# PFLeget/treegp

Measured on AMD Instinct MI355X. Metric: GP solve+predict throughput, 2-D AnisotropicRBF N=65536, higher is better.
Workload: dtype f64

## Files before the change

treegp_amd/csrc/api.hip:

```cpp
#include "tgp_internal.h"

#include <chrono>

namespace {
struct Arena {
    char *base;
    size_t off = 0;
    template <typename T> T *take(size_t count) {
        T *p = reinterpret_cast<T *>(base + off);
        off += (count * sizeof(T) + 255) / 256 * 256;
        return p;
    }
};

struct Staging {
    void *buf = nullptr;
    size_t bytes = 0;
};
Staging g_dummy;
}

struct tgp_ctx_ext {
    Staging io;
    Staging hio;
// ... 321 lines not shown
    double *d_out = (double *)ext_of(ctx)->io.buf;
    rc = launch_unpack_lower(ctx, d_A, Np, n, d_out);
    if (rc) return rc;
    TGP_HIP(hipMemcpyAsync(out, d_out, (size_t)n * n * sizeof(double), hipMemcpyDeviceToHost, ctx->stream));
    TGP_HIP(hipStreamSynchronize(ctx->stream));
    return 0;
}

int tgp_factor_device(tgp_ctx *ctx, const tgp_factor *f, const double **d_A, const double **d_W, int64_t *Np) {
    TGP_ARG(f && d_A && d_W && Np);
    *d_A = f->d_A;
    *d_W = f->d_W;
    *Np = f->Np;
    return 0;
}

static int factor_and_solve(tgp_ctx *ctx, int64_t n, int64_t Np, const double *d_y, double *d_alpha, double *logdet,
                            double *ydota, tgp_factor **keep, bool augmented) {
    hipStream_t st = ctx->stream;
    tgp_ctx_ext *e = ext_of(ctx);
    double *d_A = e->A_cache, *d_W = e->W_cache;
    double *d_b = (double *)ctx->scratch;
    int rc = 0;
    static const bool both_sweeps = getenv("TGP_CHI2_BOTH_SWEEPS") != nullptr;
    const bool forward_only = d_alpha == nullptr && !both_sweeps;
    double *own_slabs = nullptr;
    int own_S = 0;
    auto fail = [&](int code) {
        if (own_slabs) (void)hipFree(own_slabs);
        return code;
    };
    static const bool dbg = getenv("TGP_HOST_PHASES") != nullptr;
    const auto h0 = std::chrono::steady_clock::now();
    int info = launch_potrf(ctx, d_A, Np, d_W, true, n);
    if (info < 0) return fail(info);
    const auto h1 = std::chrono::steady_clock::now();
    TGP_HIP(hipEventRecord(ctx->ev[2], st));
    double sweeps = 0.0;
    if (info == 0 && augmented) {
        rc = launch_logdet_rowsq(ctx, d_A, Np, n, ctx->d_scal);
        if (rc) return fail(rc);
        if (d_alpha) {
            int Sa = 0;
            (void)potrs_big_step(Np, &Sa);
            rc = tgp_ensure_scratch2(ctx, (size_t)Np * sizeof(double));
            if (rc) return fail(rc);
            double *d_z = (double *)ctx->scratch2, *slabs = nullptr;
            bool build = false;
            rc = acquire_slabs(ctx, Np, Sa, nullptr, nullptr, &slabs, &build);
            if (rc) return fail(rc);
            rc = launch_vslab_build(ctx, d_A, d_W, Np, Sa, slabs);
            if (rc) return fail(rc);
            rc = launch_extract_row(ctx, d_A, Np, n, d_z);
            if (rc) return fail(rc);
            rc = launch_potrs_big_bwd(ctx, d_A, Np, Sa, slabs, d_b, d_z);
            if (rc) return fail(rc);
            sweeps = 1.0;
            TGP_HIP(hipMemcpyAsync(d_alpha, d_b, (size_t)n * sizeof(double), hipMemcpyDeviceToDevice, st));
        }
        TGP_HIP(hipMemcpyAsync(ctx->h_scal, ctx->d_scal, 2 * sizeof(double), hipMemcpyDeviceToHost, st));
    } else if (info == 0) {
        rc = launch_pad_copy(ctx, d_y, n, Np, d_b);
        if (rc) return fail(rc);
        int S2 = 0;
        if (keep && !own_slabs && potrs_big_step(Np, &S2) && ctx->vslab && ctx->vslab_bytes == vslab_bytes(Np, S2)) {
            own_slabs = (double *)ctx->vslab;
            own_S = S2;
            ctx->vslab = nullptr;
            ctx->vslab_bytes = 0;
        }
        if (own_slabs) {
            rc = launch_vslab_build(ctx, d_A, d_W, Np, own_S, own_slabs);
            if (rc) return fail(rc);
        }
        rc = launch_potrs(ctx, d_A, d_W, Np, d_b, forward_only, keep ? &own_slabs : nullptr, keep ? &own_S : nullptr);
        if (rc) return fail(rc);
        sweeps = forward_only ? 1.0 : 2.0;
        rc = launch_logdet_dot(ctx, d_A, Np, n, forward_only ? d_b : d_y, d_b, ctx->d_scal);
        if (rc) return fail(rc);
        if (d_alpha) TGP_HIP(hipMemcpyAsync(d_alpha, d_b, (size_t)n * sizeof(double), hipMemcpyDeviceToDevice, st));
        TGP_HIP(hipMemcpyAsync(ctx->h_scal, ctx->d_scal, 2 * sizeof(double), hipMemcpyDeviceToHost, st));
    }
    TGP_HIP(hipEventRecord(ctx->ev[3], st));
    const auto h2 = std::chrono::steady_clock::now();
    TGP_HIP(hipStreamSynchronize(st));
    if (dbg) {
        const auto h3 = std::chrono::steady_clock::now();
        auto d = [](std::chrono::steady_clock::time_point a, std::chrono::steady_clock::time_point b) { return std::chrono::duration<double, std::milli>(b - a).count(); };
        fprintf(stderr, "[factor_and_solve] launch_potrf returned after %.2f ms, solves queued after %.2f ms, final sync %.2f ms\n", d(h0, h1), d(h1, h2), d(h2, h3));
    }
    if (info == 0) info = *ctx->h_info;
    if (info < 0) return fail(tgp_potrf_info_rc(ctx, info));
    float ms = 0.f;
    TGP_HIP(hipEventElapsedTime(&ms, ctx->ev[0], ctx->ev[1]));
    ctx->timings[0] = ms;
    TGP_HIP(hipEventElapsedTime(&ms, ctx->ev[1], ctx->ev[2]));
    ctx->timings[1] = ms;
    TGP_HIP(hipEventElapsedTime(&ms, ctx->ev[2], ctx->ev[3]));
    ctx->timings[2] = ms;
    ctx->timings[8] = 8.0 * ((double)Np * (Np + 1) / 2.0) + 16.0 * (double)Np;
    ctx->timings[10] = sweeps;
    if (info > 0) {
        if (info > n) info = (int)n;
        return fail(info);
    }
    if (logdet) *logdet = ctx->h_scal[0];
    if (ydota) *ydota = ctx->h_scal[1];
    if (keep) {
        tgp_factor *f = new tgp_factor();
        f->n = n;
        f->Np = Np;
        f->d_A = d_A;
        f->d_W = d_W;
        f->d_slabs = own_slabs;
        f->slab_S = own_S;
        e->A_cache = e->W_cache = nullptr;
        e->cache_Np = 0;
        *keep = f;
    }
    return 0;
}

static int gp_solve_once(tgp_ctx *ctx, const tgp_kernel *k, const double *d_X, int64_t n, const double *d_y,
                         const double *d_yerr, double *d_alpha, double *logdet, double *ydota, tgp_factor **keep);
int tgp_d_gp_solve(tgp_ctx *ctx, const tgp_kernel *k, const double *d_X, int64_t n, const double *d_y,
                   const double *d_yerr, double *d_alpha, double *logdet, double *ydota, tgp_factor **keep) {
    SolveInFlight here;
    ctx->mid_allowed = here.alone ? 1 : 0;
    int rc = gp_solve_once(ctx, k, d_X, n, d_y, d_yerr, d_alpha, logdet, ydota, keep);
    ctx->mid_allowed = 0;
    if (rc == TGP_RC_HANDOFF && !ctx->mid_off) {
        ctx->mid_off = 1;
        rc = gp_solve_once(ctx, k, d_X, n, d_y, d_yerr, d_alpha, logdet, ydota, keep);
    }
    return rc;
}
// ... 298 lines not shown
```

treegp_amd/csrc/chol.hip:

```cpp
#include "tgp_internal.h"

#include "gemm_tile.h"
#include "potrf128.h"

#ifdef TGP_POTRF_STAMPS
__device__ unsigned long long tgp_gemm_stamps[1024 * 4];
__device__ int tgp_gemm_stamp_grid = 43;
__device__ unsigned long long tgp_queue_stamps[1024 * 4];
__device__ int tgp_queue_stamp_T = 40;
__device__ unsigned long long tgp_mid_stamps[25 * 8];
__device__ int tgp_mid_stamp_base = 5120;
#define TGP_MID_STAMP(i)                                                                                   \
    do {                                                                                                   \
        if (threadIdx.x == 0 && base == tgp_mid_stamp_base && blockIdx.x < 25) tgp_mid_stamps[blockIdx.x * 8 + (i)] = __builtin_amdgcn_s_memrealtime(); \
    } while (0)
#else
#define TGP_MID_STAMP(i) ((void)0)
#endif

namespace {
template <int MODE, int LDB>
__global__ __launch_bounds__(256, 2) void gemm_col_kernel(const double *A, const double *B, double *C) {
    const int64_t t = blockIdx.x;
    TGP_CHAIN_PRIO();
// ... 556 lines not shown
    static const int strip32_t = [] { const char *e = getenv("TGP_STRIP32_T"); return e ? atoi(e) : 64; }();
    if (strip > 0 && T <= strip32_t) {
        syrk_strip32_kernel<NSEG><<<(unsigned)((int64_t)4 * T * strip), 256, 0, st>>>(d_A, Np, ob, T, strip, P0, P1);
        return;
    }
    if (strip > 0 && T <= strip64_t) {
        syrk_strip64_kernel<NSEG><<<(unsigned)((int64_t)2 * T * strip), 256, 0, st>>>(d_A, Np, ob, T, strip, P0, P1);
        return;
    }
    const unsigned gs = strip == 0 ? (unsigned)tilemap_grid(T) : (unsigned)((int64_t)T * strip);
    syrk_dtv_kernel<NSEG><<<gs, 256, 0, st>>>(d_A, Np, ob, T, strip, P0, P1);
}

int queued_nres(int T) {
    static const int queue_res = [] { const char *e = getenv("TGP_QUEUE_RES"); return e ? atoi(e) : 0; }();
    if (queue_res > 0) return queue_res > TGP_QUEUE_MAXRES ? TGP_QUEUE_MAXRES : queue_res;
    static const int t1 = [] { const char *e = getenv("TGP_QUEUE_T1"); return e ? atoi(e) : 42; }();
    static const int t2 = [] { const char *e = getenv("TGP_QUEUE_T2"); return e ? atoi(e) : 26; }();
    return T >= t1 ? 1 : (T >= t2 ? 2 : 3);
}
void launch_syrk2_queued(tgp_ctx *ctx, hipStream_t st, double *d_A, int64_t Np, int ob, int T, const double *P0, const double *P1,
                         int nqueue) {
    const int nres = queued_nres(T);
    static const int half_env = [] { const char *e = getenv("TGP_QUEUE_HALF"); return e ? atoi(e) : -1; }();
    const unsigned slots = (unsigned)(tilemap_grid(T) / 8);
    unsigned nhalf = half_env >= 0 ? (unsigned)half_env : (unsigned)(512 - 64 * nres) / 8u;
    if (nhalf > slots) nhalf = slots;
    static const int steal = [] { const char *e = getenv("TGP_QUEUE_STEAL"); return e ? atoi(e) : 1; }();
    syrk_dtv_queue_kernel<2><<<512 + 8, 256, 0, st>>>(d_A, Np, ob, T, slots + nhalf, slots - nhalf, nres,
                                                     ctx->d_queue + TGP_QUEUE_WORDS * nqueue, P0, P1, steal);
}
}

int launch_potrf(tgp_ctx *ctx, double *d_A, int64_t Np, double *d_W, bool defer_info, int64_t n_data) {
    TGP_ARG(Np > 0 && Np % TGP_PW == 0);
    hipStream_t st = ctx->stream;
    TGP_HIP(hipMemsetAsync(ctx->d_info, 0, sizeof(int), st));
    const int nP = (int)(Np / TGP_PW);
    const bool prof = ctx->profiling != 0;
    if (prof) {
        while ((int)ctx->prof_events.size() < 2 * nP) {
            hipEvent_t e;
            TGP_HIP(hipEventCreate(&e));
            ctx->prof_events.push_back(e);
        }
    }
    static const int mode_env = [] { const char *e = getenv("TGP_CHOL_MODE"); return e ? atoi(e) : -1; }();
    const int mode = mode_env >= 0 ? mode_env : (!ctx->lookahead ? 1 : (Np >= 18432 ? 3 : (Np <= 1280 ? 1 : 2)));
    if (mode >= 2) {
        int rc = tgp_ensure_side_stream(ctx);
        if (rc) return rc;
    }
    double flops = 0.0;
    int nlaunch = 0;
    bool counting = true;
    auto timed = [&](auto &&fn, double fl) -> int {
        if (!counting) {
            fn();
            return 0;
        }
        if (prof) TGP_HIP(hipEventRecord(ctx->prof_events[2 * nlaunch], st));
        fn();
        if (prof) TGP_HIP(hipEventRecord(ctx->prof_events[2 * nlaunch + 1], st));
        flops += fl;
        ++nlaunch;
        return 0;
    };
    auto Wk = [&](int k) { return d_W + (int64_t)(2 * k) * TGP_TB * TGP_TB; };
// ... 109 lines not shown
                    syrk_small_kernel<2><<<dim3((unsigned)(T * 8), (unsigned)cols), 256, 0, st>>>(
                        d_A, Np, ob, T, seg_rows(k0 + i, ob), seg_rows(k0 + i + 1, ob));
                return;
            }
            SegPtrs<4> P{{seg_rows(k0, ob), seg_rows(k0 + 1, ob), seg_rows(k0 + 2, ob), seg_rows(k0 + 3, ob)},
                         {nullptr, nullptr, nullptr, nullptr}};
            const unsigned gs = strip == 0 ? (unsigned)tilemap_grid(T) : (unsigned)((int64_t)T * strip);
            syrk_segs_kernel<4><<<gs, 256, 0, st>>>(d_A, Np, ob, T, strip, P);
        };
        static const int tail_tiles = [] { const char *e = getenv("TGP_QUAD_TAIL_TILES"); return e ? atoi(e) : 96; }();
        factor_group(st, 0);
        for (int k = 0; k + 4 < nP; k += 4) {
            const int T4 = (int)((Np - (int64_t)TGP_PW * (k + 4)) / TGP_TB);
            if (T4 <= tail_tiles) {
                const double m = (double)T4 * TGP_TB;
                int rc = timed([&] { bulk(k, k + 4, T4, 0); }, 4.0 * TGP_PW * m * (m + 1.0));
                if (rc) return rc;
                counting = false;
                rc = run_pairs(k + 4);
                counting = true;
                if (rc) return rc;
                break;
            }
            {
                const double rows = (double)T4 * TGP_TB, w = (T4 < 8 ? T4 : 8) * (double)TGP_TB;
                const double elems = w * (rows - w) + w * (w + 1.0) / 2.0;
                int rc = timed([&] { bulk(k, k + 4, T4, 8); }, 2.0 * 4.0 * TGP_PW * elems);
                if (rc) return rc;
            }
            TGP_HIP(tgp_signal(ctx, st, 0, ctx->ev[4]));
            TGP_HIP(tgp_await(ctx, sd, 0, ctx->ev[4]));
            factor_group(sd, k + 4);
            TGP_HIP(tgp_signal(ctx, sd, 1, ctx->ev[5]));
            const int T5 = T4 - 8;
            if (T5 > 0) {
                const double m = (double)T5 * TGP_TB;
                int rc = timed([&] { bulk(k, k + 8, T5, 0); }, 4.0 * TGP_PW * m * (m + 1.0));
                if (rc) return rc;
            }
            TGP_HIP(tgp_await(ctx, st, 1, ctx->ev[5]));
        }
    } else if (mode == 2) {
        int rc = run_pairs(0);
        if (rc) return rc;
    } else {
        for (int k = 0; k < nP; k += 2) {
            const int64_t mk = Np - (int64_t)TGP_PW * k;
            factor_panel(st, panel(k), mk, Wk(k), ctx->d_info, k * TGP_PW, false, n_data, psync(k), 256);
            if (k + 1 >= nP) break;
            const int T1 = (int)((mk - TGP_PW) / TGP_TB);
            launch_syrk<1>(st, d_A, Np, k + 1, T1, 2, panel(k) + (int64_t)TGP_PW * TGP_PW, nullptr);
            factor_panel(st, panel(k + 1), mk - TGP_PW, Wk(k + 1), ctx->d_info, (k + 1) * TGP_PW, false, n_data, psync(k + 1), 256);
            const int T2 = T1 - 2;
            if (T2 > 0) {
                const double m = (double)T2 * TGP_TB;
                int rc = timed([&] { launch_syrk<2>(st, d_A, Np, k + 2, T2, 0, panel(k) + (int64_t)2 * TGP_PW * TGP_PW,
                                                     panel(k + 1) + (int64_t)TGP_PW * TGP_PW); },
                               2.0 * TGP_PW * m * (m + 1.0));
                if (rc) return rc;
            }
        }
    }
    TGP_HIP(hipGetLastError());
    TGP_HIP(hipMemcpyAsync(ctx->h_info, ctx->d_info, sizeof(int), hipMemcpyDeviceToHost, st));
    ctx->timings[6] = nlaunch;
    ctx->timings[7] = flops;
    ctx->timings[5] = 0.0;
    if (defer_info && !prof) return 0;
    TGP_HIP(hipStreamSynchronize(st));
    if (prof) {
        double tot = 0.0;
        for (int i = 0; i < nlaunch; ++i) {
            float ms = 0.f;
// ... 213 lines not shown
```

treegp_amd/csrc/tgp_internal.h:

```cpp
#pragma once
#include <hip/hip_runtime.h>
#include <cstdint>
#include <cstdio>
#include <cstdlib>
#include <cstring>
#include <string>
#include <atomic>
#include <vector>
#include "../../include/tgp.h"

#ifdef TGP_NO_CHAIN_PRIO
#define TGP_CHAIN_PRIO() ((void)0)
#else
#define TGP_CHAIN_PRIO() __builtin_amdgcn_s_setprio(3)
#endif

#define TGP_QUEUE_MAXRES 6
#define TGP_QUEUE_LEAVE (8 + 32 * TGP_QUEUE_MAXRES)
#define TGP_QUEUE_WORDS (TGP_QUEUE_LEAVE + 8)
#define TGP_NQUEUE 128
#define TGP_PSYNC_PANELS 1024
#define TGP_TB 128
#define TGP_PW 256
#define TGP_VAR_CHUNK_MAX 65280
// ... 117 lines not shown
    const int64_t S = (T + (1 << sh) - 1) >> sh;
    const int64_t ns = S * (S + 1) / 2;
    const int per = 1 << (2 * sh), q = per >= 8 ? per / 8 : 1;
    const int xcd = (int)(b & 7);
    const int64_t slot = b >> 3;
    const int64_t whole = (ns / 8) * per;
    int64_t st;
    int within;
    if (slot < whole) {
        st = (slot >> (2 * sh)) * 8 + xcd;
        within = (int)(slot & (per - 1));
    } else {
        const int64_t nn = slot - whole;
        st = (ns / 8) * 8 + nn / q;
        within = xcd * q + (int)(nn % q);
        if (st >= ns || within >= per) return;
    }
    int64_t Si, Sj;
    tri_index(st, Si, Sj);
    const int i = (int)((Si << sh) + (within >> sh));
    const int j = (int)((Sj << sh) + (within & ((1 << sh) - 1)));
    if (j > i || i >= T) return;
    ti = i; tj = j;
}

int tgp_ensure_side_stream(tgp_ctx *ctx);
int tgp_ensure_scratch(tgp_ctx *ctx, size_t bytes);
int tgp_ensure_scratch2(tgp_ctx *ctx, size_t bytes);
int tgp_ensure_pinned(tgp_ctx *ctx, size_t bytes, void **out);
int launch_kbuild_lower(tgp_ctx *ctx, const tgp_kernel *k, const double *d_X, int64_t n, int64_t Np,
                        const double *d_yerr, double *d_A);
int launch_kernel_dense(tgp_ctx *ctx, const tgp_kernel *k, const double *d_X, int64_t n,
                        const double *d_Y, int64_t m, int self, double *d_out);
int launch_potrf(tgp_ctx *ctx, double *d_A, int64_t Np, double *d_W, bool defer_info = false, int64_t n_data = -1);
int tgp_potrf_info_rc(tgp_ctx *ctx, int info);
#define TGP_RC_HANDOFF (-4)
extern std::atomic<int> tgp_solves_in_flight;
#define TGP_FLAG_HEAD 8
#define TGP_FLAG_HEAD_COUNT 9
bool tgp_handoff_by_flags(tgp_ctx *ctx);
unsigned tgp_next_seq(tgp_ctx *ctx, int id, hipError_t *err);
hipError_t tgp_signal_value(tgp_ctx *ctx, hipStream_t from, int id, unsigned v);
hipError_t tgp_signal(tgp_ctx *ctx, hipStream_t from, int id, hipEvent_t ev);
hipError_t tgp_await(tgp_ctx *ctx, hipStream_t to, int id, hipEvent_t ev);
bool potrs_big_step(int64_t Np, int *S);
int acquire_slabs(tgp_ctx *ctx, int64_t Np, int S, double **slab_cache, int *slab_S, double **out, bool *need_build);
int launch_potrs_big_bwd(tgp_ctx *ctx, const double *d_A, int64_t Np, int S, const double *slabs, double *d_b, double *d_z);
int launch_kbuild_lower_dist(tgp_ctx *ctx, const tgp_kernel *k, const double *d_X, int64_t n, int64_t Np,
                             const double *d_yerr, double *d_Aloc, const int64_t *d_loff, int G, int g);
int launch_factor_diag256(tgp_ctx *ctx, double *blk, double *W0, double *W1, int base, bool latency = false);
int launch_trsm_rows(tgp_ctx *ctx, double *rows, int ntiles, const double *Lkk, const double *W0, const double *W1, double *keepW = nullptr);
int launch_syrk_distn(tgp_ctx *ctx, double *d_Aloc, const int64_t *d_loff, int64_t Np, int kpanel, int G, int g, int nseg,
                      const double *const *d_P, const int *cmax, int col_lo, int col_hi, int queue_nres = 0, int head_cols = 0,
                      const double *const *d_PB = nullptr);
int launch_diag256_fwd(tgp_ctx *ctx, const double *Lkk, const double *W0, const double *W1, double *y);
int launch_diag256_bwd(tgp_ctx *ctx, const double *Lkk, const double *W0, const double *W1, double *y, const double *s);
int launch_fwd_update_rows(tgp_ctx *ctx, const double *Lrows, int64_t rows, const double *z, double *yrows);
int launch_gemv_t_rows(tgp_ctx *ctx, const double *Lrows, int64_t rows, const double *a, double *s, int64_t max_rows);
int launch_logdet_dist(tgp_ctx *ctx, const double *d_Aloc, const int64_t *d_loff, int64_t Np, int64_t n, int G, int g,
                       double *d_out);
int launch_potrs(tgp_ctx *ctx, const double *d_A, const double *d_W, int64_t Np, double *d_b, bool forward_only = false,
                 double **slab_cache = nullptr, int *slab_S = nullptr);
int launch_potrs_128(tgp_ctx *ctx, const double *d_A, const double *d_W, int64_t Np, double *d_b, bool forward_only);
size_t vslab_bytes(int64_t Np, int S);
int factor_slabs(tgp_ctx *ctx, tgp_factor *f, int want_S, int *S, const double **slabs);
int tgp_ensure_io(tgp_ctx *ctx, size_t bytes);
void *tgp_io_buffer(tgp_ctx *ctx);
void tgp_factor_release_to_cache(tgp_ctx *ctx, tgp_factor *f);
int launch_loglik_grad(tgp_ctx *ctx, tgp_factor *f, const tgp_kernel *k, const double *d_X, const double *d_alpha, double *grad);
int launch_vslab_build(tgp_ctx *ctx, const double *d_A, const double *d_W, int64_t Np, int S, double *slabs);
struct SlabPipeline {
    int chunk;
    hipEvent_t ready[16];
};
int launch_vslab_build_range(tgp_ctx *ctx, hipStream_t st, const double *d_A, const double *d_W, int64_t Np, int S, double *slabs,
                             int64_t row_lo, int64_t row_hi);
int launch_potrs_big(tgp_ctx *ctx, const double *d_A, int64_t Np, int S, const double *slabs, double *d_b, double *d_z,
                     bool forward_only, const SlabPipeline *pipe = nullptr);
int launch_potrs_big_multi(tgp_ctx *ctx, const double *d_A, int64_t Np, int S, const double *slabs, double *d_B, double *d_Z, int nrhs);
int launch_logdet(tgp_ctx *ctx, const double *d_A, int64_t Np, int64_t n, double *d_out);
int launch_dot(tgp_ctx *ctx, const double *d_a, const double *d_b, int64_t n, double *d_out);
int launch_logdet_dot(tgp_ctx *ctx, const double *d_A, int64_t Np, int64_t n, const double *d_a, const double *d_b, double *d_out);
int launch_pad_copy(tgp_ctx *ctx, const double *d_y, int64_t n, int64_t Np, double *d_b);
int launch_augment_rhs(tgp_ctx *ctx, double *d_A, int64_t Np, int64_t n, const double *d_y);
int launch_extract_row(tgp_ctx *ctx, const double *d_A, int64_t Np, int64_t n, double *d_z);
int launch_logdet_rowsq(tgp_ctx *ctx, const double *d_A, int64_t Np, int64_t n, double *d_out);
int launch_predict(tgp_ctx *ctx, const tgp_kernel *k, const double *d_X, int64_t n, const double *d_alpha,
                   const double *d_Xs, int64_t m, double *d_ys);
int launch_unpack_lower(tgp_ctx *ctx, const double *d_A, int64_t Np, int64_t n, double *d_out);
int launch_pack_lower(tgp_ctx *ctx, const double *d_K, int64_t n, int64_t Np, const double *d_yerr, double *d_A);
int launch_potrs_multi(tgp_ctx *ctx, const double *d_A, const double *d_W, int64_t Np, double *d_B, int nrhs, double **slab_cache,
                       int *slab_S = nullptr);
size_t lmul_partial_bytes(int64_t Np, int nrhs);
int launch_factor_lmul(tgp_ctx *ctx, const double *d_A, int64_t Np, const double *d_Z, int nrhs, double *d_Y, double *d_partial);
```

treegp_amd/csrc/trsv.hip:

```cpp
#include "tgp_internal.h"

namespace {
__device__ __forceinline__ double wave_sum(double v) {
#pragma unroll
    for (int o = 32; o > 0; o >>= 1) v += __shfl_down(v, o, 64);
    return v;
}

__global__ __launch_bounds__(256) void diag_gemv_n_kernel(const double *__restrict__ W, double *y) {
    __shared__ double M[128 * 129];
    __shared__ double ys[128], part[256];
    const int tid = threadIdx.x;
    {
        const int c = (tid & 63) * 2, r0 = tid >> 6;
        double2 v[32];
#pragma unroll
        for (int k = 0; k < 32; ++k) v[k] = *reinterpret_cast<const double2 *>(W + (r0 + 4 * k) * 128 + c);
        if (tid < 128) ys[tid] = y[tid];
#pragma unroll
        for (int k = 0; k < 32; ++k) {
            M[(r0 + 4 * k) * 129 + c] = v[k].x;
            M[(r0 + 4 * k) * 129 + c + 1] = v[k].y;
        }
    }
// ... 343 lines not shown
    TGP_HIP(hipStreamWaitEvent(sd, ctx->ev_slab[16], 0));
    rc = launch_vslab_build_range(ctx, st, d_A, d_W, Np, S, slabs, 0, (int64_t)pipe->chunk * S);
    if (rc) return rc;
    for (int c = 1; c * pipe->chunk < nS; ++c) {
        rc = launch_vslab_build_range(ctx, sd, d_A, d_W, Np, S, slabs, (int64_t)c * pipe->chunk * S, (int64_t)(c + 1) * pipe->chunk * S);
        if (rc) return rc;
        pipe->ready[c] = ctx->ev_slab[c];
        TGP_HIP(hipEventRecord(pipe->ready[c], sd));
    }
    return 0;
}

int factor_slabs(tgp_ctx *ctx, tgp_factor *f, int want_S, int *S, const double **slabs) {
    *slabs = nullptr;
    *S = 0;
    int step;
    if (!potrs_big_config(f->Np, &step)) return 0;
    const bool own = want_S && want_S != step && !getenv("TGP_POTRS_STEP");
    if (own) step = want_S;
    double *sl = nullptr;
    bool build = false;
    int rc = acquire_slabs(ctx, f->Np, step, own ? &f->d_slabs2 : &f->d_slabs, own ? &f->slab2_S : &f->slab_S, &sl, &build);
    if (rc) return rc;
    if (build) {
        rc = launch_vslab_build(ctx, f->d_A, f->d_W, f->Np, step, sl);
        if (rc) return rc;
    }
    *S = step;
    *slabs = sl;
    return 0;
}

int launch_potrs(tgp_ctx *ctx, const double *d_A, const double *d_W, int64_t Np, double *d_b, bool forward_only,
                 double **slab_cache, int *slab_S) {
    int S;
    if (!potrs_big_config(Np, &S)) return launch_potrs_128(ctx, d_A, d_W, Np, d_b, forward_only);
    int rc = tgp_ensure_scratch2(ctx, (size_t)Np * sizeof(double));
    if (rc) return rc;
    double *slabs = nullptr;
    bool build = false, piped = false;
    rc = acquire_slabs(ctx, Np, S, slab_cache, slab_S, &slabs, &build);
    if (rc) return rc;
    SlabPipeline pipe;
    if (build) {
        rc = build_slabs_pipelined(ctx, d_A, d_W, Np, S, slabs, &pipe, &piped);
        if (rc) return rc;
    }
    return launch_potrs_big(ctx, d_A, Np, S, slabs, d_b, (double *)ctx->scratch2, forward_only, piped ? &pipe : nullptr);
}

int launch_potrs_multi(tgp_ctx *ctx, const double *d_A, const double *d_W, int64_t Np, double *d_B, int nrhs, double **slab_cache,
                       int *slab_S) {
    int S;
    if (!potrs_big_config(Np, &S)) {
        for (int v = 0; v < nrhs; ++v) {
            int rc = launch_potrs_128(ctx, d_A, d_W, Np, d_B + (int64_t)v * Np, false);
            if (rc) return rc;
        }
        return 0;
    }
    int rc = tgp_ensure_scratch2(ctx, (size_t)nrhs * Np * sizeof(double));
    if (rc) return rc;
    double *slabs = nullptr;
    bool build = false;
    rc = acquire_slabs(ctx, Np, S, slab_cache, slab_S, &slabs, &build);
    if (rc) return rc;
    if (build) {
        rc = launch_vslab_build(ctx, d_A, d_W, Np, S, slabs);
        if (rc) return rc;
    }
    return launch_potrs_big_multi(ctx, d_A, Np, S, slabs, d_B, (double *)ctx->scratch2, nrhs);
}

int launch_potrs_128(tgp_ctx *ctx, const double *d_A, const double *d_W, int64_t Np, double *d_b, bool forward_only) {
    hipStream_t st = ctx->stream;
    const int nb = (int)(Np / TGP_TB);
    for (int kb = 0; kb < nb; ++kb) {
// ... 134 lines not shown
```

treegp_amd/csrc/trsv_big.hip:

```cpp
#include "tgp_internal.h"
#include "gemm_tile.h"

namespace {
__device__ __forceinline__ double wsum(double v) {
#pragma unroll
    for (int o = 32; o > 0; o >>= 1) v += __shfl_down(v, o, 64);
    return v;
}
__device__ __forceinline__ int64_t slab_off(int64_t Np, int64_t row, int lcol) {
    return (int64_t)(lcol >> 8) * Np * 256 + row * 256 + (lcol & 255);
}

__global__ __launch_bounds__(256) void vinit_kernel(const double *__restrict__ W, double *__restrict__ V, double *__restrict__ Vt,
                                                    int64_t Np, int S, int boff) {
    __shared__ double T[128 * 129];
    const int tid = threadIdx.x;
    const int blk = blockIdx.x + boff;
    const int64_t r0 = (int64_t)blk * 128;
    const int lc0 = (int)(r0 % S);
    const bool odd = (blk & 1) != 0;
    const double *src = W + r0 * 128;
    const int c = (tid & 63) * 2, rr = tid >> 6;
    const double2 zero = make_double2(0.0, 0.0);
#pragma unroll 8
// ... 158 lines not shown
#pragma unroll
        for (int v = 0; v < NR; ++v) {
            zr[v][q][0] = *reinterpret_cast<const double2 *>(z + v * vs + qq * 256 + 2 * lane);
            zr[v][q][1] = *reinterpret_cast<const double2 *>(z + v * vs + qq * 256 + 128 + 2 * lane);
            if (q >= npan) zr[v][q][0] = zr[v][q][1] = make_double2(0.0, 0.0);
        }
#pragma unroll
        for (int t = 0; t < RPW; ++t) {
            const int64_t r = first + t;
            const int64_t rr = row0 + (r < nrows ? r : nrows - 1);
            av[t][q][0] = *reinterpret_cast<const double2 *>(base + rr * TGP_PW);
            av[t][q][1] = *reinterpret_cast<const double2 *>(base + rr * TGP_PW + 128);
        }
    }
    double mysum = 0.0;
#pragma unroll
    for (int v = 0; v < NR; ++v)
#pragma unroll
        for (int t = 0; t < RPW; ++t) {
            double acc = 0.0;
#pragma unroll
            for (int q = 0; q < NP; ++q)
                acc += (av[t][q][0].x * zr[v][q][0].x + av[t][q][0].y * zr[v][q][0].y) +
                       (av[t][q][1].x * zr[v][q][1].x + av[t][q][1].y * zr[v][q][1].y);
#pragma unroll
            for (int o = 32; o > 0; o >>= 1) acc += __shfl_xor(acc, o, 64);
            if (lane == v * RPW + t) mysum = acc;
        }
    if (lane < NR * RPW && mine < nrows) b[myv * vs + row0 + mine] = bold - mysum;
}

template <int CW, int NR>
__global__ __launch_bounds__(512) void bulk_bwd_kernel(const double *__restrict__ A, int64_t Np, int64_t r0, int rows,
                                                       const double *__restrict__ a, double *z, int64_t vs) {
    constexpr int LPR = CW / 2;
    constexpr int RPI = 64 / LPR;
    extern __shared__ double dyn_lds[];
    double *as = dyn_lds;
    double2 *part = reinterpret_cast<double2 *>(dyn_lds);
    const int tid = threadIdx.x, lane = tid & 63, wave = tid >> 6;
    const int sub = lane / LPR, cl = lane % LPR;
    const int64_t c0 = (int64_t)blockIdx.x * CW, p = c0 >> 8;
    const char *ubase = reinterpret_cast<const char *>(A + panel_off(p, Np) + (r0 - p * TGP_PW) * TGP_PW + (c0 & 255));
    const int loff = 16 * cl;
    const int per = rows >> 3;
    const int i0 = wave * per + sub;
    double2 zold[NR];
#pragma unroll
    for (int v = 0; v < NR; ++v) zold[v] = tid < LPR ? *reinterpret_cast<const double2 *>(z + v * vs + c0 + 2 * tid) : make_double2(0.0, 0.0);
    constexpr int U = (CW == 128 && NR == 1) ? 16 : 8, STEP = U * RPI;
    const int end = wave * per + per;
    auto ld = [&](int i, int u) {
        const int r = i + u * RPI;
        return *reinterpret_cast<const double2 *>(ubase + (unsigned)((r < end ? r : end - 1) * (TGP_PW * 8) + loff));
    };
    double2 v0[U], v1[U];
#pragma unroll
    for (int u = 0; u < U; ++u) v0[u] = ld(i0, u);
#pragma unroll
    for (int v = 0; v < NR; ++v)
        for (int i = tid; i < rows; i += 512) as[v * rows + i] = a[v * vs + r0 + i];
    __syncthreads();
    auto wt = [&](int v, int i, int u) {
        const int r = i + u * RPI;
        return r < end ? as[v * rows + r] : 0.0;
    };
    double sx[NR], sy[NR];
#pragma unroll
    for (int v = 0; v < NR; ++v) sx[v] = sy[v] = 0.0;
#pragma unroll 1
    for (int i = i0; i < end; i += 2 * STEP) {
        const bool second = i - sub + STEP < end;
        if (second) {
#pragma unroll
            for (int u = 0; u < U; ++u) v1[u] = ld(i + STEP, u);
// ... 14 lines not shown
#pragma unroll
            for (int u = 0; u < U; ++u)
#pragma unroll
                for (int v = 0; v < NR; ++v) {
                    const double w = wt(v, i + STEP, u);
                    sx[v] += v1[u].x * w;
                    sy[v] += v1[u].y * w;
                }
        }
    }
    __syncthreads();
#pragma unroll
    for (int v = 0; v < NR; ++v) {
#pragma unroll
        for (int o = 32; o >= LPR; o >>= 1) {
            sx[v] += __shfl_xor(sx[v], o, 64);
            sy[v] += __shfl_xor(sy[v], o, 64);
        }
        if (lane < LPR) part[(v * 8 + wave) * LPR + lane] = make_double2(sx[v], sy[v]);
    }
    __syncthreads();
    if (tid < LPR) {
#pragma unroll
        for (int v = 0; v < NR; ++v) {
            double tx = 0.0, ty = 0.0;
#pragma unroll
            for (int w = 0; w < 8; ++w) { tx += part[(v * 8 + w) * LPR + tid].x; ty += part[(v * 8 + w) * LPR + tid].y; }
            zold[v].x -= tx;
            zold[v].y -= ty;
            *reinterpret_cast<double2 *>(z + v * vs + c0 + 2 * tid) = zold[v];
        }
    }
}
}

size_t vslab_bytes(int64_t Np, int S) { return (size_t)2 * Np * S * sizeof(double); }

int launch_vslab_build_range(tgp_ctx *ctx, hipStream_t st, const double *d_A, const double *d_W, int64_t Np, int S, double *slabs,
                             int64_t row_lo, int64_t row_hi) {
    const size_t tt_need = (size_t)Np * S * sizeof(double);
    if (tt_need > ctx->vslab_tt_bytes) {
        TGP_HIP(hipDeviceSynchronize());
        if (ctx->vslab_tt) TGP_HIP(hipFree(ctx->vslab_tt));
        ctx->vslab_tt = nullptr;
        ctx->vslab_tt_bytes = 0;
        TGP_HIP(hipMalloc(&ctx->vslab_tt, tt_need));
        ctx->vslab_tt_bytes = tt_need;
    }
    double *V = slabs, *Vt = slabs + Np * S, *TT = (double *)ctx->vslab_tt;
    if (row_hi > Np) row_hi = Np;
    if (row_hi <= row_lo) return 0;
    const int64_t span = row_hi - row_lo;
    vinit_kernel<<<(unsigned)(span / 128), 256, 0, st>>>(d_W, V, Vt, Np, S, (int)(row_lo / 128));
    static const int64_t small_below = getenv("TGP_VSLAB_SMALL_BELOW") ? atoll(getenv("TGP_VSLAB_SMALL_BELOW")) : 12288;
    for (int h = 128; h < S && h < Np; h *= 2) {
        const int nt = h / 128;
        const unsigned nq = (unsigned)((span + 2 * h - 1) / (2 * h));
        const int qoff = (int)(row_lo / (2 * h));
        const unsigned grid = nq * nt * nt;
        const bool small = Np < small_below && h <= 512;
        const unsigned sgrid = nq * nt * (h / 16);
        if (h == 128) {
            if (small) {
                vprod_small_kernel<128, false><<<sgrid, 256, 0, st>>>(d_A, V, Vt, TT, Np, S, h, qoff);
                vprod_small_kernel<128, true><<<sgrid, 256, 0, st>>>(d_A, V, Vt, TT, Np, S, h, qoff);
            } else {
// ... 4 lines not shown
            vprod_small_kernel<256, false><<<sgrid, 256, 0, st>>>(d_A, V, Vt, TT, Np, S, h, qoff);
            vprod_small_kernel<256, true><<<sgrid, 256, 0, st>>>(d_A, V, Vt, TT, Np, S, h, qoff);
        } else {
            vprod_kernel<256, false><<<grid, 256, 0, st>>>(d_A, V, Vt, TT, Np, S, h, qoff);
            vprod_kernel<256, true><<<grid, 256, 0, st>>>(d_A, V, Vt, TT, Np, S, h, qoff);
        }
        vtrans_kernel<<<grid, 256, 0, st>>>(V, Vt, Np, S, h, qoff);
    }
    TGP_HIP(hipGetLastError());
    return 0;
}

int launch_vslab_build(tgp_ctx *ctx, const double *d_A, const double *d_W, int64_t Np, int S, double *slabs) {
    return launch_vslab_build_range(ctx, ctx->stream, d_A, d_W, Np, S, slabs, 0, Np);
}

namespace {
template <bool UPPER, int NR>
void launch_diag_gemv(hipStream_t st, int NPmax, const double *M, int64_t Np, int64_t r0, int rows, const double *in, double *out,
                      int64_t vs) {
    const unsigned grid = (unsigned)((rows + 3) / 4);
    if (NPmax <= 2) diag_gemv_big_kernel<UPPER, 2, NR><<<grid, 256, 0, st>>>(M, Np, r0, rows, in, out, vs);
    else diag_gemv_big_kernel<UPPER, 4, NR><<<grid, 256, 0, st>>>(M, Np, r0, rows, in, out, vs);
}

template <int NP, int NR>
void launch_bulk_fwd(hipStream_t st, const double *d_A, int64_t Np, int p0, int npan, int64_t row0, int64_t below, const double *z,
                     double *b, int64_t vs) {
    constexpr int RPW = (16 / NP) / (NR > 1 ? 2 : 1) > 0 ? (16 / NP) / (NR > 1 ? 2 : 1) : 1;
    bulk_fwd_kernel<NP, NR><<<(unsigned)((below + 4 * RPW - 1) / (4 * RPW)), 256, 0, st>>>(d_A, Np, p0, npan, row0, below, z, b, vs);
}

template <int NR>
void fwd_step(hipStream_t st, const double *d_A, int64_t Np, int S, const double *V, int K, double *d_b, double *d_z, int64_t vs) {
    const int NPmax = S / 256;
    const int64_t r0 = (int64_t)K * S;
    const int rows = (int)((Np - r0) < S ? (Np - r0) : S);
    launch_diag_gemv<false, NR>(st, NPmax, V, Np, r0, rows, d_b, d_z, vs);
    const int64_t below = Np - (r0 + rows);
    if (below > 0) {
        const int p0 = (int)(r0 / 256), npan = rows / 256;
        if (NPmax <= 2) launch_bulk_fwd<2, NR>(st, d_A, Np, p0, npan, r0 + rows, below, d_z + r0, d_b, vs);
        else launch_bulk_fwd<4, NR>(st, d_A, Np, p0, npan, r0 + rows, below, d_z + r0, d_b, vs);
    }
}

template <int NR>
int potrs_big_nr(tgp_ctx *ctx, const double *d_A, int64_t Np, int S, const double *slabs, double *d_b, double *d_z, int64_t vs,
                 bool forward_only, const SlabPipeline *pipe = nullptr, bool backward_only = false) {
    hipStream_t st = ctx->stream;
    const double *V = slabs, *Vt = slabs + Np * S;
    const int nS = (int)((Np + S - 1) / S);
    const int NPmax = S / 256;
    for (int K = 0; K < nS && !backward_only; ++K) {
        if (pipe && K > 0 && K % pipe->chunk == 0) TGP_HIP(hipStreamWaitEvent(st, pipe->ready[K / pipe->chunk], 0));
        fwd_step<NR>(st, d_A, Np, S, V, K, d_b, d_z, vs);
    }
    if (forward_only) {
        for (int v = 0; v < NR; ++v)
            TGP_HIP(hipMemcpyAsync(d_b + v * vs, d_z + v * vs, (size_t)Np * sizeof(double), hipMemcpyDeviceToDevice, st));
        TGP_HIP(hipGetLastError());
        return 0;
    }
    for (int K = nS - 1; K >= 0; --K) {
        const int64_t r0 = (int64_t)K * S;
        const int rows = (int)((Np - r0) < S ? (Np - r0) : S);
        launch_diag_gemv<true, NR>(st, NPmax, Vt, Np, r0, rows, d_z, d_b, vs);
        if (K > 0) {
            if (r0 / 128 >= 512) {
                const size_t lds = (size_t)NR * (rows * 8 > 8 * 64 * 16 ? rows * 8 : 8 * 64 * 16);
                bulk_bwd_kernel<128, NR><<<(unsigned)(r0 / 128), 512, lds, st>>>(d_A, Np, r0, rows, d_b, d_z, vs);
            } else {
                const size_t lds = (size_t)NR * (rows * 8 > 8 * 16 * 16 ? rows * 8 : 8 * 16 * 16);
                bulk_bwd_kernel<32, NR><<<(unsigned)(r0 / 32), 512, lds, st>>>(d_A, Np, r0, rows, d_b, d_z, vs);
            }
        }
    }
    TGP_HIP(hipGetLastError());
    return 0;
}
}

int launch_potrs_big(tgp_ctx *ctx, const double *d_A, int64_t Np, int S, const double *slabs, double *d_b, double *d_z,
                     bool forward_only, const SlabPipeline *pipe) {
    return potrs_big_nr<1>(ctx, d_A, Np, S, slabs, d_b, d_z, Np, forward_only, pipe);
}

int launch_potrs_big_bwd(tgp_ctx *ctx, const double *d_A, int64_t Np, int S, const double *slabs, double *d_b, double *d_z) {
    return potrs_big_nr<1>(ctx, d_A, Np, S, slabs, d_b, d_z, Np, false, nullptr, true);
}

int launch_potrs_big_multi(tgp_ctx *ctx, const double *d_A, int64_t Np, int S, const double *slabs, double *d_B, double *d_Z, int nrhs) {
    int v = 0, rc = 0;
    for (; v + 4 <= nrhs && !rc; v += 4) rc = potrs_big_nr<4>(ctx, d_A, Np, S, slabs, d_B + (int64_t)v * Np, d_Z + (int64_t)v * Np, Np, false);
    for (; v + 2 <= nrhs && !rc; v += 2) rc = potrs_big_nr<2>(ctx, d_A, Np, S, slabs, d_B + (int64_t)v * Np, d_Z + (int64_t)v * Np, Np, false);
    for (; v < nrhs && !rc; ++v) rc = potrs_big_nr<1>(ctx, d_A, Np, S, slabs, d_B + (int64_t)v * Np, d_Z + (int64_t)v * Np, Np, false);
    return rc;
}
```

Before: 243,300.

## Overlap slab build with factorization and add lookahead split in triangular sweeps

Two overlaps are added. Building the inverse diagonal-block slabs now happens incrementally on the side stream during the Cholesky factorization, so the solve phase only builds the remaining rows. The forward and backward blocked triangular sweeps also use a lookahead split: the side stream updates the next block's rows and runs its diagonal solve while the main stream finishes the rest of the bulk update. This trades extra streams, events and launches for shorter critical-path latency, and adds risk of races or extra sync overhead.

```diff
diff --git a/treegp_amd/csrc/api.hip b/treegp_amd/csrc/api.hip
--- a/treegp_amd/csrc/api.hip
+++ b/treegp_amd/csrc/api.hip
@@ -377,7 +377,28 @@
     };
     static const bool dbg = getenv("TGP_HOST_PHASES") != nullptr;
     const auto h0 = std::chrono::steady_clock::now();
-    int info = launch_potrf(ctx, d_A, Np, d_W, true, n);
+    SideSlabs ss{nullptr, 0, 0};
+    int Sb = 0;
+    if ((!augmented || d_alpha) && tgp_sweep_lookahead_on() && ctx->lookahead && tgp_solves_in_flight.load() <= 1 &&
+        potrs_big_step(Np, &Sb) && Sb == 1024) {
+        if (keep && !augmented) {
+            if (ctx->vslab && ctx->vslab_bytes == vslab_bytes(Np, Sb)) {
+                own_slabs = (double *)ctx->vslab;
+                ctx->vslab = nullptr;
+                ctx->vslab_bytes = 0;
+            } else {
+                TGP_HIP(hipMalloc((void **)&own_slabs, vslab_bytes(Np, Sb)));
+            }
+            own_S = Sb;
+            ss.slabs = own_slabs;
+        } else {
+            bool build = false;
+            rc = acquire_slabs(ctx, Np, Sb, nullptr, nullptr, &ss.slabs, &build);
+            if (rc) return fail(rc);
+        }
+        ss.S = Sb;
+    }
+    int info = launch_potrf(ctx, d_A, Np, d_W, true, n, ss.slabs ? &ss : nullptr);
     if (info < 0) return fail(info);
     const auto h1 = std::chrono::steady_clock::now();
     TGP_HIP(hipEventRecord(ctx->ev[2], st));
@@ -394,7 +415,7 @@
             bool build = false;
             rc = acquire_slabs(ctx, Np, Sa, nullptr, nullptr, &slabs, &build);
             if (rc) return fail(rc);
-            rc = launch_vslab_build(ctx, d_A, d_W, Np, Sa, slabs);
+            rc = launch_vslab_build_range(ctx, st, d_A, d_W, Np, Sa, slabs, slabs == ss.slabs ? ss.built_rows : 0, Np);
             if (rc) return fail(rc);
             rc = launch_extract_row(ctx, d_A, Np, n, d_z);
             if (rc) return fail(rc);
@@ -415,10 +436,10 @@
             ctx->vslab_bytes = 0;
         }
         if (own_slabs) {
-            rc = launch_vslab_build(ctx, d_A, d_W, Np, own_S, own_slabs);
+            rc = launch_vslab_build_range(ctx, st, d_A, d_W, Np, own_S, own_slabs, own_slabs == ss.slabs ? ss.built_rows : 0, Np);
             if (rc) return fail(rc);
         }
-        rc = launch_potrs(ctx, d_A, d_W, Np, d_b, forward_only, keep ? &own_slabs : nullptr, keep ? &own_S : nullptr);
+        rc = launch_potrs(ctx, d_A, d_W, Np, d_b, forward_only, keep ? &own_slabs : nullptr, keep ? &own_S : nullptr, ss.built_rows);
         if (rc) return fail(rc);
         sweeps = forward_only ? 1.0 : 2.0;
         rc = launch_logdet_dot(ctx, d_A, Np, n, forward_only ? d_b : d_y, d_b, ctx->d_scal);
@@ -447,6 +468,7 @@
     ctx->timings[10] = sweeps;
     if (info > 0) {
         if (info > n) info = (int)n;
+        ctx->err = "Cholesky: the leading minor of order " + std::to_string(info) + " is not positive definite";
         return fail(info);
     }
     if (logdet) *logdet = ctx->h_scal[0];
diff --git a/treegp_amd/csrc/chol.hip b/treegp_amd/csrc/chol.hip
--- a/treegp_amd/csrc/chol.hip
+++ b/treegp_amd/csrc/chol.hip
@@ -612,8 +612,9 @@
 }
 }
 
-int launch_potrf(tgp_ctx *ctx, double *d_A, int64_t Np, double *d_W, bool defer_info, int64_t n_data) {
+int launch_potrf(tgp_ctx *ctx, double *d_A, int64_t Np, double *d_W, bool defer_info, int64_t n_data, SideSlabs *side_slabs) {
     TGP_ARG(Np > 0 && Np % TGP_PW == 0);
+    if (side_slabs) side_slabs->built_rows = 0;
     hipStream_t st = ctx->stream;
     TGP_HIP(hipMemsetAsync(ctx->d_info, 0, sizeof(int), st));
     const int nP = (int)(Np / TGP_PW);
@@ -789,6 +790,12 @@
             TGP_HIP(tgp_await(ctx, sd, 0, ctx->ev[4]));
             factor_group(sd, k + 4);
             TGP_HIP(tgp_signal(ctx, sd, 1, ctx->ev[5]));
+            if (side_slabs && side_slabs->S == 4 * TGP_PW) {
+                const int64_t lo = k == 0 ? 0 : (int64_t)TGP_PW * (k + 4), hi = (int64_t)TGP_PW * (k + 8) < Np ? (int64_t)TGP_PW * (k + 8) : Np;
+                int rc = launch_vslab_build_range(ctx, sd, d_A, d_W, Np, side_slabs->S, side_slabs->slabs, lo, hi);
+                if (rc) return rc;
+                side_slabs->built_rows = hi;
+            }
             const int T5 = T4 - 8;
             if (T5 > 0) {
                 const double m = (double)T5 * TGP_TB;
@@ -796,6 +803,10 @@
                 if (rc) return rc;
             }
             TGP_HIP(tgp_await(ctx, st, 1, ctx->ev[5]));
+        }
+        if (side_slabs && side_slabs->built_rows > 0) {
+            TGP_HIP(tgp_signal(ctx, sd, 3, ctx->ev[7]));
+            TGP_HIP(tgp_await(ctx, st, 3, ctx->ev[7]));
         }
     } else if (mode == 2) {
         int rc = run_pairs(0);
diff --git a/treegp_amd/csrc/tgp_internal.h b/treegp_amd/csrc/tgp_internal.h
--- a/treegp_amd/csrc/tgp_internal.h
+++ b/treegp_amd/csrc/tgp_internal.h
@@ -173,7 +173,13 @@
                         const double *d_yerr, double *d_A);
 int launch_kernel_dense(tgp_ctx *ctx, const tgp_kernel *k, const double *d_X, int64_t n,
                         const double *d_Y, int64_t m, int self, double *d_out);
-int launch_potrf(tgp_ctx *ctx, double *d_A, int64_t Np, double *d_W, bool defer_info = false, int64_t n_data = -1);
+struct SideSlabs {
+    double *slabs;
+    int S;
+    int64_t built_rows;
+};
+int launch_potrf(tgp_ctx *ctx, double *d_A, int64_t Np, double *d_W, bool defer_info = false, int64_t n_data = -1,
+                 SideSlabs *side_slabs = nullptr);
 int tgp_potrf_info_rc(tgp_ctx *ctx, int info);
 #define TGP_RC_HANDOFF (-4)
 extern std::atomic<int> tgp_solves_in_flight;
@@ -185,6 +191,7 @@
 hipError_t tgp_signal(tgp_ctx *ctx, hipStream_t from, int id, hipEvent_t ev);
 hipError_t tgp_await(tgp_ctx *ctx, hipStream_t to, int id, hipEvent_t ev);
 bool potrs_big_step(int64_t Np, int *S);
+bool tgp_sweep_lookahead_on();
 int acquire_slabs(tgp_ctx *ctx, int64_t Np, int S, double **slab_cache, int *slab_S, double **out, bool *need_build);
 int launch_potrs_big_bwd(tgp_ctx *ctx, const double *d_A, int64_t Np, int S, const double *slabs, double *d_b, double *d_z);
 int launch_kbuild_lower_dist(tgp_ctx *ctx, const tgp_kernel *k, const double *d_X, int64_t n, int64_t Np,
@@ -201,7 +208,7 @@
 int launch_logdet_dist(tgp_ctx *ctx, const double *d_Aloc, const int64_t *d_loff, int64_t Np, int64_t n, int G, int g,
                        double *d_out);
 int launch_potrs(tgp_ctx *ctx, const double *d_A, const double *d_W, int64_t Np, double *d_b, bool forward_only = false,
-                 double **slab_cache = nullptr, int *slab_S = nullptr);
+                 double **slab_cache = nullptr, int *slab_S = nullptr, int64_t built_rows = 0);
 int launch_potrs_128(tgp_ctx *ctx, const double *d_A, const double *d_W, int64_t Np, double *d_b, bool forward_only);
 size_t vslab_bytes(int64_t Np, int S);
 int factor_slabs(tgp_ctx *ctx, tgp_factor *f, int want_S, int *S, const double **slabs);
diff --git a/treegp_amd/csrc/trsv.hip b/treegp_amd/csrc/trsv.hip
--- a/treegp_amd/csrc/trsv.hip
+++ b/treegp_amd/csrc/trsv.hip
@@ -399,7 +399,7 @@
 }
 
 int launch_potrs(tgp_ctx *ctx, const double *d_A, const double *d_W, int64_t Np, double *d_b, bool forward_only,
-                 double **slab_cache, int *slab_S) {
+                 double **slab_cache, int *slab_S, int64_t built_rows) {
     int S;
     if (!potrs_big_config(Np, &S)) return launch_potrs_128(ctx, d_A, d_W, Np, d_b, forward_only);
     int rc = tgp_ensure_scratch2(ctx, (size_t)Np * sizeof(double));
@@ -409,7 +409,10 @@
     rc = acquire_slabs(ctx, Np, S, slab_cache, slab_S, &slabs, &build);
     if (rc) return rc;
     SlabPipeline pipe;
-    if (build) {
+    if (build && built_rows > 0) {
+        rc = launch_vslab_build_range(ctx, ctx->stream, d_A, d_W, Np, S, slabs, built_rows, Np);
+        if (rc) return rc;
+    } else if (build) {
         rc = build_slabs_pipelined(ctx, d_A, d_W, Np, S, slabs, &pipe, &piped);
         if (rc) return rc;
     }
diff --git a/treegp_amd/csrc/trsv_big.hip b/treegp_amd/csrc/trsv_big.hip
--- a/treegp_amd/csrc/trsv_big.hip
+++ b/treegp_amd/csrc/trsv_big.hip
@@ -214,7 +214,7 @@
 
 template <int CW, int NR>
 __global__ __launch_bounds__(512) void bulk_bwd_kernel(const double *__restrict__ A, int64_t Np, int64_t r0, int rows,
-                                                       const double *__restrict__ a, double *z, int64_t vs) {
+                                                       const double *__restrict__ a, double *z, int64_t vs, int cb) {
     constexpr int LPR = CW / 2;
     constexpr int RPI = 64 / LPR;
     extern __shared__ double dyn_lds[];
@@ -222,7 +222,7 @@
     double2 *part = reinterpret_cast<double2 *>(dyn_lds);
     const int tid = threadIdx.x, lane = tid & 63, wave = tid >> 6;
     const int sub = lane / LPR, cl = lane % LPR;
-    const int64_t c0 = (int64_t)blockIdx.x * CW, p = c0 >> 8;
+    const int64_t c0 = (int64_t)(blockIdx.x + cb) * CW, p = c0 >> 8;
     const char *ubase = reinterpret_cast<const char *>(A + panel_off(p, Np) + (r0 - p * TGP_PW) * TGP_PW + (c0 & 255));
     const int loff = 16 * cl;
     const int per = rows >> 3;
@@ -303,6 +303,11 @@
         }
     }
 }
+}
+
+bool tgp_sweep_lookahead_on() {
+    static const bool on = !(getenv("TGP_SWEEP_LOOKAHEAD") && atoi(getenv("TGP_SWEEP_LOOKAHEAD")) == 0);
+    return on;
 }
 
 size_t vslab_bytes(int64_t Np, int S) { return (size_t)2 * Np * S * sizeof(double); }
@@ -373,18 +378,54 @@
 }
 
 template <int NR>
-void fwd_step(hipStream_t st, const double *d_A, int64_t Np, int S, const double *V, int K, double *d_b, double *d_z, int64_t vs) {
+void fwd_bulk(hipStream_t st, const double *d_A, int64_t Np, int S, int K, int64_t row0, int64_t nrows, double *d_b, double *d_z, int64_t vs) {
     const int NPmax = S / 256;
     const int64_t r0 = (int64_t)K * S;
     const int rows = (int)((Np - r0) < S ? (Np - r0) : S);
-    launch_diag_gemv<false, NR>(st, NPmax, V, Np, r0, rows, d_b, d_z, vs);
+    const int p0 = (int)(r0 / 256), npan = rows / 256;
+    if (NPmax <= 2) launch_bulk_fwd<2, NR>(st, d_A, Np, p0, npan, row0, nrows, d_z + r0, d_b, vs);
+    else launch_bulk_fwd<4, NR>(st, d_A, Np, p0, npan, row0, nrows, d_z + r0, d_b, vs);
+}
+
+template <int NR>
+void fwd_diag(hipStream_t st, int64_t Np, int S, const double *V, int K, double *d_b, double *d_z, int64_t vs) {
+    const int64_t r0 = (int64_t)K * S;
+    const int rows = (int)((Np - r0) < S ? (Np - r0) : S);
+    launch_diag_gemv<false, NR>(st, S / 256, V, Np, r0, rows, d_b, d_z, vs);
+}
+
+template <int NR>
+void fwd_step(hipStream_t st, const double *d_A, int64_t Np, int S, const double *V, int K, double *d_b, double *d_z, int64_t vs) {
+    const int64_t r0 = (int64_t)K * S;
+    const int rows = (int)((Np - r0) < S ? (Np - r0) : S);
+    fwd_diag<NR>(st, Np, S, V, K, d_b, d_z, vs);
     const int64_t below = Np - (r0 + rows);
-    if (below > 0) {
-        const int p0 = (int)(r0 / 256), npan = rows / 256;
-        if (NPmax <= 2) launch_bulk_fwd<2, NR>(st, d_A, Np, p0, npan, r0 + rows, below, d_z + r0, d_b, vs);
-        else launch_bulk_fwd<4, NR>(st, d_A, Np, p0, npan, r0 + rows, below, d_z + r0, d_b, vs);
-    }
-}
+    if (below > 0) fwd_bulk<NR>(st, d_A, Np, S, K, r0 + rows, below, d_b, d_z, vs);
+}
+
+template <int NR>
+void bwd_diag(hipStream_t st, int64_t Np, int S, const double *Vt, int K, double *d_b, double *d_z, int64_t vs) {
+    const int64_t r0 = (int64_t)K * S;
+    const int rows = (int)((Np - r0) < S ? (Np - r0) : S);
+    launch_diag_gemv<true, NR>(st, S / 256, Vt, Np, r0, rows, d_z, d_b, vs);
+}
+
+template <int NR>
+void bwd_bulk(hipStream_t st, const double *d_A, int64_t Np, int S, int K, int64_t c_lo, int64_t c_hi, double *d_b, double *d_z, int64_t vs) {
+    const int64_t r0 = (int64_t)K * S;
+    const int rows = (int)((Np - r0) < S ? (Np - r0) : S);
+    if (r0 / 128 >= 512) {
+        const size_t lds = (size_t)NR * (rows * 8 > 8 * 64 * 16 ? rows * 8 : 8 * 64 * 16);
+        bulk_bwd_kernel<128, NR><<<(unsigned)((c_hi - c_lo) / 128), 512, lds, st>>>(d_A, Np, r0, rows, d_b, d_z, vs, (int)(c_lo / 128));
+    } else {
+        const size_t lds = (size_t)NR * (rows * 8 > 8 * 16 * 16 ? rows * 8 : 8 * 16 * 16);
+        bulk_bwd_kernel<32, NR><<<(unsigned)((c_hi - c_lo) / 32), 512, lds, st>>>(d_A, Np, r0, rows, d_b, d_z, vs, (int)(c_lo / 32));
+    }
+}
+
+constexpr int FLAG_SWEEP_A = 4, FLAG_SWEEP_B = 5;
+constexpr int64_t SWEEP_SPLIT_FWD_ROWS = 12288, SWEEP_SPLIT_BWD_COLS = 12288;
+
 
 template <int NR>
 int potrs_big_nr(tgp_ctx *ctx, const double *d_A, int64_t Np, int S, const double *slabs, double *d_b, double *d_z, int64_t vs,
@@ -392,10 +433,40 @@
     hipStream_t st = ctx->stream;
     const double *V = slabs, *Vt = slabs + Np * S;
     const int nS = (int)((Np + S - 1) / S);
-    const int NPmax = S / 256;
+    const int64_t fwd_min = SWEEP_SPLIT_FWD_ROWS, bwd_min = SWEEP_SPLIT_BWD_COLS;
+    bool la = tgp_sweep_lookahead_on() && ctx->lookahead && !pipe && S == 1024 && tgp_solves_in_flight.load() <= 1 &&
+              Np - 2 * (int64_t)S >= (fwd_min < bwd_min ? fwd_min : bwd_min);
+    hipStream_t sd = nullptr;
+    if (la) {
+        int rc = tgp_ensure_side_stream(ctx);
+        if (rc) return rc;
+        sd = ctx->side_stream;
+        for (int i = 12; i < 14; ++i)
+            if (!ctx->ev_slab[i]) TGP_HIP(hipEventCreateWithFlags(&ctx->ev_slab[i], hipEventDisableTiming));
+    }
+    hipEvent_t evA = ctx->ev_slab[12], evB = ctx->ev_slab[13];
+    bool have = false;
     for (int K = 0; K < nS && !backward_only; ++K) {
         if (pipe && K > 0 && K % pipe->chunk == 0) TGP_HIP(hipStreamWaitEvent(st, pipe->ready[K / pipe->chunk], 0));
-        fwd_step<NR>(st, d_A, Np, S, V, K, d_b, d_z, vs);
+        const int64_t r0 = (int64_t)K * S;
+        const int rows = (int)((Np - r0) < S ? (Np - r0) : S);
+        const int64_t below = Np - (r0 + rows);
+        const int64_t nrows1 = below < S ? below : S;
+        const bool split = la && below - nrows1 >= fwd_min;
+        if (!have) fwd_diag<NR>(st, Np, S, V, K, d_b, d_z, vs);
+        if (!split) {
+            if (below > 0) fwd_bulk<NR>(st, d_A, Np, S, K, r0 + rows, below, d_b, d_z, vs);
+            have = false;
+            continue;
+        }
+        TGP_HIP(tgp_signal(ctx, st, FLAG_SWEEP_B, evB));
+        TGP_HIP(tgp_await(ctx, sd, FLAG_SWEEP_B, evB));
+        fwd_bulk<NR>(sd, d_A, Np, S, K, r0 + rows, nrows1, d_b, d_z, vs);
+        fwd_diag<NR>(sd, Np, S, V, K + 1, d_b, d_z, vs);
+        TGP_HIP(tgp_signal(ctx, sd, FLAG_SWEEP_A, evA));
+        fwd_bulk<NR>(st, d_A, Np, S, K, r0 + rows + nrows1, below - nrows1, d_b, d_z, vs);
+        TGP_HIP(tgp_await(ctx, st, FLAG_SWEEP_A, evA));
+        have = true;
     }
     if (forward_only) {
         for (int v = 0; v < NR; ++v)
@@ -403,19 +474,24 @@
         TGP_HIP(hipGetLastError());
         return 0;
     }
+    have = false;
     for (int K = nS - 1; K >= 0; --K) {
         const int64_t r0 = (int64_t)K * S;
-        const int rows = (int)((Np - r0) < S ? (Np - r0) : S);
-        launch_diag_gemv<true, NR>(st, NPmax, Vt, Np, r0, rows, d_z, d_b, vs);
-        if (K > 0) {
-            if (r0 / 128 >= 512) {
-                const size_t lds = (size_t)NR * (rows * 8 > 8 * 64 * 16 ? rows * 8 : 8 * 64 * 16);
-                bulk_bwd_kernel<128, NR><<<(unsigned)(r0 / 128), 512, lds, st>>>(d_A, Np, r0, rows, d_b, d_z, vs);
-            } else {
-                const size_t lds = (size_t)NR * (rows * 8 > 8 * 16 * 16 ? rows * 8 : 8 * 16 * 16);
-                bulk_bwd_kernel<32, NR><<<(unsigned)(r0 / 32), 512, lds, st>>>(d_A, Np, r0, rows, d_b, d_z, vs);
-            }
-        }
+        const bool split = la && K >= 2 && r0 - S >= bwd_min;
+        if (!have) bwd_diag<NR>(st, Np, S, Vt, K, d_b, d_z, vs);
+        if (!split) {
+            if (K > 0) bwd_bulk<NR>(st, d_A, Np, S, K, 0, r0, d_b, d_z, vs);
+            have = false;
+            continue;
+        }
+        TGP_HIP(tgp_signal(ctx, st, FLAG_SWEEP_B, evB));
+        TGP_HIP(tgp_await(ctx, sd, FLAG_SWEEP_B, evB));
+        bwd_bulk<NR>(sd, d_A, Np, S, K, r0 - S, r0, d_b, d_z, vs);
+        bwd_diag<NR>(sd, Np, S, Vt, K - 1, d_b, d_z, vs);
+        TGP_HIP(tgp_signal(ctx, sd, FLAG_SWEEP_A, evA));
+        bwd_bulk<NR>(st, d_A, Np, S, K, 0, r0 - S, d_b, d_z, vs);
+        TGP_HIP(tgp_await(ctx, st, FLAG_SWEEP_A, evA));
+        have = true;
     }
     TGP_HIP(hipGetLastError());
     return 0;
```

After: 238,600. -1.9%, worse.
